# mklawonn/Scene-Graph-GAN

Hardware: AMD Instinct MI355X
Metric: triples/sec (G+D step) (higher is better)
Workload: dtype f32 (conv operands scaled per tensor and split into 2 fp16 pieces, round-to-nearest = 23 significant bits, 3 fp16 MFMAs per product, f32 accumulate; native-f32 figure and parity in the same line); 1 GPU; BASELINE.json configs[1] (1xMI355X, batch 64, 224x224, vocab 1000): batch 64 per GPU, 224x224 synthetic images, vocab 1000, 3-token triples, 1 critic update + 1 generator update per step (WGAN-GP lambda=10, TF-Adam); global_batch=64, critic_iters=1, parallelism=dp1, conv_precision_mode=2, schedule=two-stream; per-kernel figures from serial steps

## Files before the change

scene-graph-gan_amd/build.py:

```python
from __future__ import annotations

import hashlib
import os
import subprocess
import sys
from concurrent.futures import ThreadPoolExecutor

HERE = os.path.dirname(os.path.abspath(__file__))
CSRC = os.path.join(HERE, "csrc")
OUT_DIR = os.path.join(HERE, "_build")
LIB_PATH = os.path.join(HERE, "libsgg_hip.so")
ARCH = "gfx950"
HIPCC = os.environ.get("HIPCC", "/opt/rocm/bin/hipcc")
NO_PACKED_FP32 = ["-Xclang", "-target-feature", "-Xclang", "-packed-fp32-ops"]
FLAGS = ["-O3", "-std=c++17", "-fPIC", "--offload-arch=" + ARCH, "-fno-gpu-rdc", "-Wall", "-Wno-unused-function",
         "-ffp-contract=fast"] + NO_PACKED_FP32


def sources():
    return sorted(os.path.join(CSRC, f) for f in os.listdir(CSRC) if f.endswith(".hip"))


def _digest(paths):
    h = hashlib.sha256()
    for p in sorted(paths):
        with open(p, "rb") as f:
            h.update(p.encode())
            h.update(f.read())
    h.update(" ".join(FLAGS).encode())
    return h.hexdigest()


def _compile(src):
    obj = os.path.join(OUT_DIR, os.path.basename(src) + ".o")
    cmd = [HIPCC] + FLAGS + ["-I", CSRC, "-c", src, "-o", obj]
    r = subprocess.run(cmd, capture_output=True, text=True)
    if r.returncode != 0:
        raise RuntimeError("hipcc failed for %s:\n%s\n%s" % (src, r.stdout, r.stderr))
    err = "\n".join(l for l in r.stderr.splitlines() if "is not a recognized feature for this target" not in l)
    return obj, err


OBJDUMP = os.environ.get("LLVM_OBJDUMP", os.path.join(os.path.dirname(os.path.dirname(os.path.realpath(HIPCC))), "lib", "llvm", "bin",
                                                      "llvm-objdump"))


M0_ASM_KERNELS = ("conv_wgrad_dma", "conv_s2_kernel")


def check_device_code(lib_path: str = LIB_PATH) -> int:
    import re
    import shutil
    tmp = os.path.join(OUT_DIR, "disasm")
    shutil.rmtree(tmp, ignore_errors=True)
    os.makedirs(tmp)
    copy = os.path.join(tmp, "lib.so")
    shutil.copy(lib_path, copy)
    if not os.path.exists(OBJDUMP):
        raise RuntimeError("llvm-objdump not found at %s (set LLVM_OBJDUMP): the build cannot verify that the library is free of "
                           "packed-fp32 VALU instructions" % OBJDUMP)
    r = subprocess.run([OBJDUMP, "--offloading", copy], capture_output=True, text=True)
    if r.returncode != 0:
        raise RuntimeError("llvm-objdump --offloading failed:\n%s" % r.stderr)
    objs = sorted(f for f in os.listdir(tmp) if f.endswith(ARCH))
    if not objs:
        raise RuntimeError("no %s code object found in %s" % (ARCH, lib_path))
    pat, n_ins, bad = re.compile(r"\bv_pk_[a-z0-9]+_f32\b"), 0, []
    sym_pat = re.compile(r"^[0-9a-f]+ <(\S+)>:")
    m0_ok = re.compile(r"^\s*s_mov_b32 m0, s\d+\b")
    m0_implicit = re.compile(r"\b(v_movrel[sd]*_b32|s_movrel[sd]_b(32|64)|v_readlane_b32 \S+, \S+, m0|v_writelane_b32 \S+, \S+, m0|s_sendmsg|ds_gws_\w+|"
                             r"v_interp_\w+|s_load_\w+ .*\bm0\b)")
    m0_bad, m0_seen, cur = [], 0, ""
    for f in objs:
        d = subprocess.run([OBJDUMP, "-d", os.path.join(tmp, f)], capture_output=True, text=True)
        if d.returncode != 0:
            raise RuntimeError("llvm-objdump -d failed on %s:\n%s" % (f, d.stderr))
        for line in d.stdout.splitlines():
            m = sym_pat.match(line)
            if m:
                cur = m.group(1)
# ... 58 lines not shown
```

scene-graph-gan_amd/csrc/conv_halo.h:

```cpp
#pragma once
#include "sgg_common.h"

struct HaloParams {
  const float* src;
  const void* wfrag;
  const float* bias;
  float* out;
  const float* amax_src;
  const float* amax_w;
  float* tile_stats;
  const float* ln_stats;
  const float* ln_gamma;
  const float* ln_beta;
  int B, H, W, C, N;
  int bh, bw, nblk;
  int flip;
  unsigned src_bytes, w_bytes;
  int gx;
  int in_rs, in_ps, in_cA, in_cB;
  int out_rs, out_ps, out_nA, out_nB;
  int ln_nc;
  int frag16;
  int src_s16;
  int cu_cap;
// ... 16 lines not shown
int sgg_halo_pc64_applicable(int C, int N, int precision);
void sgg_halo_pc_launch(const HaloParams& p, int precision, hipStream_t st);

struct WgradHaloPlan {
  int ct, nt;
  int nbs;
  int spw;
  int pairs, pairs_n;
  int nsplit;
  int stages;
  int nslabs;
  int geo;
  int R, pc, xslots;
  size_t ws_bytes;
};
int sgg_wgrad_halo_plan(int B, int H, int W, int Cin, int Cout, int KH, int KW, int stride, WgradHaloPlan* pl);
void sgg_wgrad_halo_launch(const float* x, const float* dy, float* slabs, int B, int H, int W, int Cin, int Cout, int stride,
                           int pad_t, int pad_l, int precision, const float* amax_x, const float* amax_dy, const WgradHaloPlan& pl,
                           hipStream_t st, const float* ln_stats = nullptr, const float* ln_gamma = nullptr,
                           const float* ln_beta = nullptr, int operand_format = 0);

struct WgradDmaPlan {
  int nt;
  int spw;
  int pairs, pairs_n;
  int nsplit, stages, nslabs;
  int geo, R, pc, xslots;
  size_t ws_bytes;
};
int sgg_wgrad_dma_plan(int B, int H, int W, int Cin, int Cout, int KH, int KW, int stride, WgradDmaPlan* pl);
void sgg_wgrad_dma_launch(const void* x, const void* dy, float* slabs, int B, int H, int W, int Cin, int Cout, int stride, int pad_t,
                          int pad_l, const float* amax_x, const float* amax_dy, const WgradDmaPlan& pl, hipStream_t st);

struct S2Params {
  const float* src;
  const void* wfrag;
  const float* bias;
  float* out;
  const float* amax_src;
  const float* amax_w;
  float* tile_stats;
  const float* ln_stats;
  const float* ln_gamma;
  const float* ln_beta;
  int B, Ho, Wo;
  int C, N;
  int M;
  int nbands;
  int pitch;
  unsigned src_bytes, w_bytes;
  int gx;
  int src_s16;
  int ksplit;
  int cu_cap;
};
int sgg_s2_applicable(int KH, int KW, int stride, int B, int Hi, int Wi, int C, int N, int precision);
int sgg_s2_stats_per_sample(int Ho, int Wo, int N);
void sgg_s2_launch(const S2Params& p, int dgrad, int precision, hipStream_t st);
```

scene-graph-gan_amd/csrc/conv_wgrad.hip:

```cpp
#include "mma_f32.h"
#include "conv_halo.h"
#include <stdlib.h>

typedef __bf16 bf16x8 __attribute__((ext_vector_type(8)));
typedef __bf16 bf16x2 __attribute__((ext_vector_type(2)));
typedef float f32x2_t __attribute__((ext_vector_type(2)));
typedef unsigned u32x4 __attribute__((ext_vector_type(4)));

typedef _Float16 f16x8 __attribute__((ext_vector_type(8)));
typedef __fp16 fp16x2 __attribute__((ext_vector_type(2)));

template <int P, bool HALF>
__device__ __forceinline__ void split8_regs(const float (&x)[8], float scale, u32x4 (&pl)[P]) {
#pragma unroll
  for (int q = 0; q < 4; ++q) {
    float a = x[2 * q], b = x[2 * q + 1];
    if constexpr (HALF) {
      a *= scale; b *= scale;
      unsigned hi, lo;
      f16_split2(a, b, hi, lo);
      pl[0][q] = hi; pl[1][q] = lo;
    } else {
#pragma unroll
      for (int pp = 0; pp < P; ++pp) {
// ... 551 lines not shown
static WgradPlan wgrad_plan(int B, int Ho, int Wo, int Cin, int Cout, int KH, int KW) {
  WgradPlan pl;
  const long long mpix = (long long)B * Ho * Wo;
  if (Cin == 3) {
    pl.bmc = 27; pl.bnc = 32;
    pl.tiles = B * sgg_cdiv(Ho, 8) * sgg_cdiv(Wo, 32);
    pl.chunk = sgg_cdiv(pl.tiles, 1024);
    pl.nsplit = sgg_cdiv(pl.tiles, pl.chunk);
    pl.ws_bytes = (size_t)pl.nsplit * 27 * 32 * sizeof(float);
    return pl;
  }
  pl.bmc = Cin >= 128 ? 128 : Cin;
  pl.bnc = Cout >= 128 ? 128 : Cout;
  pl.tiles = (Cin / pl.bmc) * (Cout / pl.bnc);
  const int base = pl.tiles * KH * KW;
  int ns = (SGG_WGRAD_WGS + base - 1) / base;
  const long long max_ns = mpix / 512 > 0 ? mpix / 512 : 1;
  if (ns > max_ns) ns = (int)max_ns;
  if (ns < 1) ns = 1;
  pl.chunk = (int)(((mpix + ns - 1) / ns + 31) / 32 * 32);
  pl.nsplit = (int)((mpix + pl.chunk - 1) / pl.chunk);
  pl.ws_bytes = pl.nsplit > 1 ? (size_t)pl.nsplit * KH * KW * Cin * Cout * sizeof(float) : 0;
  return pl;
}

extern "C" size_t sgg_conv2d_nhwc_wgrad_workspace_bytes(int B, int Hi, int Wi, int Cin, int Ho, int Wo, int Cout, int KH,
                                                        int KW) {
  size_t need = wgrad_plan(B, Ho, Wo, Cin, Cout, KH, KW).ws_bytes;
  WgradHaloPlan hp;
  const int st_guess = (Hi == Ho && Wi == Wo) ? 1 : ((Hi == 2 * Ho && Wi == 2 * Wo) ? 2 : 0);
  if (st_guess && Cin != 3 && sgg_wgrad_halo_plan(B, Ho, Wo, Cin, Cout, KH, KW, st_guess, &hp) && hp.ws_bytes > need) need = hp.ws_bytes;
  WgradDmaPlan dp;
  if (st_guess && Cin != 3 && sgg_wgrad_dma_plan(B, Ho, Wo, Cin, Cout, KH, KW, st_guess, &dp) && dp.ws_bytes > need) need = dp.ws_bytes;
  return need;
}

extern "C" int sgg_conv2d_nhwc_wgrad_resident(int B, int Ho, int Wo, int Cin, int Cout, int KH, int KW, int stride, int precision) {
  WgradHaloPlan hp;
  if (!(sgg_prec_resident(precision) && Cin != 3 && B > 0 && sgg_wgrad_halo_plan(B, Ho, Wo, Cin, Cout, KH, KW, stride, &hp))) return 0;
  WgradDmaPlan dp;
  return (precision == 2 && sgg_wgrad_dma_plan(B, Ho, Wo, Cin, Cout, KH, KW, stride, &dp)) ? 2 : 1;
}

extern "C" int sgg_conv2d_nhwc_wgrad(const float* x, const float* dy, float* dw, int B, int Hi, int Wi, int Cin, int Ho,
                                     int Wo, int Cout, int KH, int KW, int stride, int pad_t, int pad_l, int precision, int algo,
                                     const float* amax_x, const float* amax_dy, const float* ln_stats, const float* ln_gamma,
                                     const float* ln_beta, int operand_format, void* workspace, size_t workspace_bytes, void* stream) {
  SGG_CHECK_ARG(x && dy && dw, "sgg_conv2d_nhwc_wgrad: null pointer");
  SGG_CHECK_ARG(operand_format >= 0 && operand_format <= 3 && (operand_format == 0 || (sgg_prec_half(precision) && Cin != 3 && algo == 0)) &&
                    !((operand_format & 1) && ln_stats),
                "sgg_conv2d_nhwc_wgrad: pre-split (S16) operands need precision 1 / 2 and the halo-resident kernel (algo 0); x with an LN "
                "prologue is the f32 pre-LayerNorm tensor");
  SGG_CHECK_ARG(!ln_stats || (ln_gamma && ln_beta), "sgg_conv2d_nhwc_wgrad: the LN prologue needs stats, gamma and beta");
  SGG_CHECK_ARG(algo == 0 || algo == 1, "sgg_conv2d_nhwc_wgrad: algo must be 0 (auto) or 1 (per-tap kernels only)");
  SGG_CHECK_ARG(precision == 0 || (precision >= 1 && precision <= 4) || precision == 6,
                "sgg_conv2d_nhwc_wgrad: precision must be 0, 1, 2, 3, 4 or 6");
  SGG_CHECK_ARG(!sgg_prec_half(precision) || Cin == 3 || (amax_x && amax_dy), "sgg_conv2d_nhwc_wgrad: precision 1 / 2 need the amax words");
  SGG_CHECK_ARG(!ln_stats || !sgg_prec_one(precision), "sgg_conv2d_nhwc_wgrad: the LN prologue exists in the two-piece modes (2, 3) only");
  SGG_CHECK_ARG(B > 0 && Hi > 0 && Wi > 0 && Ho > 0 && Wo > 0 && stride >= 1 && stride <= 2, "sgg_conv2d_nhwc_wgrad: bad dims");
  SGG_CHECK_ARG((long long)B * Hi * Wi * Cin < (1LL << 31) && (long long)B * Ho * Wo * Cout < (1LL << 31),
                "sgg_conv2d_nhwc_wgrad: tensor exceeds 2^31 elements");
  hipStream_t st = (hipStream_t)stream;
  const WgradPlan pl = wgrad_plan(B, Ho, Wo, Cin, Cout, KH, KW);
  if (pl.ws_bytes > 0) {
    if (!workspace || workspace_bytes < pl.ws_bytes) {
      sgg_set_error("sgg_conv2d_nhwc_wgrad: workspace too small (%zu < %zu)", workspace_bytes, pl.ws_bytes);
      return SGG_ERR_WORKSPACE;
    }
  }
  const long long nout = (long long)KH * KW * Cin * Cout;
  WgradDmaPlan dp;
  if (operand_format == 3 && precision == 2 && !ln_stats && algo == 0 && pad_t == 1 && pad_l == 1 && Hi == Ho * stride &&
      Wi == Wo * stride && sgg_wgrad_dma_plan(B, Ho, Wo, Cin, Cout, KH, KW, stride, &dp)) {
    if (!workspace || workspace_bytes < dp.ws_bytes) {
      sgg_set_error("sgg_conv2d_nhwc_wgrad: workspace too small (%zu < %zu)", workspace_bytes, dp.ws_bytes);
      return SGG_ERR_WORKSPACE;
    }
    sgg_wgrad_dma_launch(x, dy, (float*)workspace, B, Ho, Wo, Cin, Cout, stride, pad_t, pad_l, amax_x, amax_dy, dp, st);
    SGG_LAUNCH_CHECK("sgg_conv2d_nhwc_wgrad(dma)");
    launch_slab_reduce((const float*)workspace, dw, nout / 4, dp.nslabs, st);
    SGG_LAUNCH_CHECK("sgg_conv2d_nhwc_wgrad(dma reduce)");
    return SGG_OK;
  }
  WgradHaloPlan hp;
  if (sgg_prec_resident(precision) && Cin != 3 && pad_t == 1 && pad_l == 1 && Hi == Ho * stride && Wi == Wo * stride &&
      algo == 0 && sgg_wgrad_halo_plan(B, Ho, Wo, Cin, Cout, KH, KW, stride, &hp) && !(hp.geo == 1 && ln_stats)) {
    if (!workspace || workspace_bytes < hp.ws_bytes) {
      sgg_set_error("sgg_conv2d_nhwc_wgrad: workspace too small (%zu < %zu)", workspace_bytes, hp.ws_bytes);
      return SGG_ERR_WORKSPACE;
    }
    sgg_wgrad_halo_launch(x, dy, (float*)workspace, B, Ho, Wo, Cin, Cout, stride, pad_t, pad_l, precision, amax_x, amax_dy, hp, st,
                          ln_stats, ln_gamma, ln_beta, operand_format);
    SGG_LAUNCH_CHECK("sgg_conv2d_nhwc_wgrad(halo)");
    launch_slab_reduce((const float*)workspace, dw, nout / 4, hp.nslabs, st);
    SGG_LAUNCH_CHECK("sgg_conv2d_nhwc_wgrad(halo reduce)");
    return SGG_OK;
  }
  SGG_CHECK_ARG(operand_format == 0, "sgg_conv2d_nhwc_wgrad: pre-split (S16) operands are served by the halo-resident kernel only");
  SGG_CHECK_ARG(!ln_stats, "sgg_conv2d_nhwc_wgrad: the LN prologue is served by the halo-resident kernel only (3x3 stride 1 or 5x5 "
                           "stride 2 on grids divisible by 8, precision 2 or 3, algo 0)");
  if (Cin == 3) {
    SGG_CHECK_ARG(KH == 3 && KW == 3 && stride == 1 && Cout == 32, "sgg_conv2d_nhwc_wgrad: Cin=3 path needs 3x3 s1 Cout=32");
    hipLaunchKernelGGL(conv_c3_wgrad_kernel<false>, dim3(pl.nsplit), dim3(256), 0, st, x, dy, (float*)workspace, Hi, Wi, pad_t, pad_l,
                       sgg_cdiv(Wo, 32), sgg_cdiv(Ho, 8), pl.tiles, pl.chunk, C3LnArgs{nullptr, nullptr, nullptr, nullptr, nullptr, nullptr});
    SGG_LAUNCH_CHECK("sgg_conv2d_nhwc_wgrad(c3)");
    launch_slab_reduce((const float*)workspace, dw, nout / 4, pl.nsplit, st);
    SGG_LAUNCH_CHECK("sgg_conv2d_nhwc_wgrad(c3 reduce)");
    return SGG_OK;
  }
  SGG_CHECK_ARG(Cin % 32 == 0 && Cout % 32 == 0, "sgg_conv2d_nhwc_wgrad: Cin and Cout must be multiples of 32 (or Cin == 3)");
  SGG_CHECK_ARG(pl.bmc == 32 || pl.bmc == 64 || pl.bmc == 128, "sgg_conv2d_nhwc_wgrad: unsupported Cin tile");
  SGG_CHECK_ARG(pl.bnc == 32 || pl.bnc == 64 || pl.bnc == 128, "sgg_conv2d_nhwc_wgrad: unsupported Cout tile");
  WgradParams p;
  p.x = x; p.dy = dy; p.out = pl.nsplit > 1 ? (float*)workspace : dw;
// ... 62 lines not shown
```

scene-graph-gan_amd/csrc/conv_wgrad_dma.hip:

```cpp
#include "split16.h"
#include "conv_halo.h"
#include <type_traits>

typedef short wd_s16x4 __attribute__((ext_vector_type(4)));
typedef unsigned wd_u32x2 __attribute__((ext_vector_type(2)));
typedef __attribute__((address_space(3))) void* wd_lds_ptr;

typedef int wd_v4i __attribute__((ext_vector_type(4)));
__device__ __forceinline__ void wd_dma16(wd_v4i rs, unsigned lds_addr, unsigned voff, int soff) {
  asm volatile("s_mov_b32 m0, %0\n\ts_nop 0\n\tbuffer_load_dwordx4 %1, %2, %3 offen lds"
               :
               : "s"(lds_addr), "v"(voff), "s"(rs), "s"(soff)
               : "memory");
}
__device__ __forceinline__ wd_v4i wd_rsrc(const void* base, unsigned bytes) {
  const unsigned long long a = reinterpret_cast<unsigned long long>(base);
  return wd_v4i{(int)(unsigned)a, (int)((unsigned)(a >> 32) & 0xffffu), (int)bytes, 0x00020000};
}
__device__ __forceinline__ unsigned wd_lds_addr(const unsigned char* p) {
  return (unsigned)(unsigned long long)(__attribute__((address_space(3))) const unsigned char*)p;
}

__device__ __forceinline__ wd_u32x2 wd_tr16(const unsigned char* p) {
  return __builtin_bit_cast(wd_u32x2, __builtin_amdgcn_ds_read_tr16_b64_v4i16((__attribute__((address_space(3))) wd_s16x4*)p));
}

struct WgradDmaParams {
  const void* x;
  const void* dy;
  float* slabs;
  const float* amax_x;
  const float* amax_dy;
  int B, H, W, C, N;
  int Hx, Wx, sxy, cy, cx, a0y, a0x, kh0, kw0, kstep, KWt, taps_total;
  int bh, bw, nblk;
  int pairs_n;
  int stages;
  unsigned x_bytes, dy_bytes;
};

#define WD_XSUB 8192
#define WD_XPLANE (2 * WD_XSUB)
#define WD_DSUB 4096

template <int NT, int NKH, int NKW>
__global__ __launch_bounds__(512, 2) void conv_wgrad_dma_kernel(WgradDmaParams p) {
  static_assert(NT == 4 || NT == 2, "64 x 128 or 64 x 64 channel tiles");
  constexpr int NTAP = NKH * NKW;
  constexpr int DPLANE = NT * WD_DSUB;
  constexpr int BUF = 2 * WD_XPLANE + 2 * DPLANE;
  constexpr int KSW = NT == 4 ? 4 : 2;
  constexpr int SPW = NT == 4 ? 1 : 2;
  __shared__ __attribute__((aligned(1024))) unsigned char lds[2 * BUF];

// ... 363 lines not shown
```

scene-graph-gan_amd/lib.py:

```python
from __future__ import annotations

import ctypes
import os
from ctypes import c_char_p, c_float, c_int, c_longlong, c_size_t, c_void_p

import torch

_HERE = os.path.dirname(os.path.abspath(__file__))
LIB_PATH = os.path.join(_HERE, "libsgg_hip.so")

_vp, _i, _f, _sz, _ll = c_void_p, c_int, c_float, c_size_t, c_longlong

SIGNATURES = {
    "sgg_version": (_i, []),
    "sgg_last_error": (c_char_p, []),
    "sgg_device_info": (_i, [_vp, _vp, _vp, _vp, _i]),
    "sgg_hwio_to_hwoi": (_i, [_vp, _vp, _i, _i, _i, _vp]),
    "sgg_conv_split_weights": (_i, [_vp, _vp, _ll, _i, _vp, _vp]),
    "sgg_absmax": (_i, [_vp, _ll, _vp, _vp]),
    "sgg_conv_wsplit_layout": (_i, [_i] * 8),
    "sgg_conv_wsplit_layout_presplit": (_i, [_i] * 8),
    "sgg_conv_s2d_weights": (_i, [_vp, _vp, _i, _i, _vp]),
    "sgg_conv_prepare_weights": (_i, [_vp, _i, _i, _vp]),
    "sgg_conv_split_weights_frag": (_i, [_vp, _vp, _i, _i, _i, _i, _vp, _vp]),
# ... 66 lines not shown
        return _lib
    path = os.environ.get("SGG_HIP_LIB", path)
    if not os.path.exists(path):
        raise SggError("libsgg_hip.so not found at %s - run `python -c 'import __graft_entry__ as g; g.build()'` "
                       "(there is no CPU fallback)" % path)
    lib = ctypes.CDLL(path)
    for name, (res, args) in SIGNATURES.items():
        fn = getattr(lib, name)
        fn.restype = res
        fn.argtypes = args
    _lib = lib
    return lib


def same_pads(in_size: int, k: int, s: int):
    out = -(-in_size // s)
    total = max((out - 1) * s + k - in_size, 0)
    return out, total // 2, total - total // 2


def _p(t):
    return None if t is None else t.data_ptr()


def _ld(t):
    return t.stride(0) if t.shape[0] > 1 else max(t.stride(0), t.shape[1])


DEFAULT_OPTIONS = {
    "conv_precision": 2,
    "conv_halo": True,
    "halo_pc": True,
    "halo_pc64": True,
    "ln_fusion": 1,
    "presplit": True,
    "presplit_head_grad": True,
    "wgrad_late": True,
    "side_priority": 0,
    "g_early": 1,
    "g_early_cus": 28,
    "c3_ln_bwd_fused": True,
    "d_side_cus": 0,
    "fwd_cus": 0,
    "ln_fusion_skip": (),
    "ln_fusion_force": (),
    "ln_fusion_force_bwd": (),
    "ln_fusion_skip_bwd": (),
}


def options_from_env(base=None):
    opts = dict(DEFAULT_OPTIONS if base is None else base)
    for item in filter(None, os.environ.get("SGG_OPTIONS", "").split(",")):
        key, _, val = item.partition("=")
        key = key.strip()
        if key not in DEFAULT_OPTIONS:
            raise SggError("SGG_OPTIONS: unknown option %r (known: %s)" % (key, ", ".join(sorted(DEFAULT_OPTIONS))))
        d = DEFAULT_OPTIONS[key]
        if isinstance(d, bool):
            opts[key] = val.strip().lower() not in ("0", "false", "no", "off", "")
        elif isinstance(d, tuple):
            opts[key] = tuple(int(v) for v in val.split("+") if v.strip())
        else:
            opts[key] = int(val)
    return opts

# ... 200 lines not shown
        else:
            nb = 4.0 * (x.numel() + y.numel())
        self._check(self._timed(sym, flops, lambda: self.lib.sgg_conv2d_nhwc_fwd(
            _p(x), _p(w_fwd), _p(w_split), _p(bias), _p(y), *d, self.conv_precision, w_split_layout, _p(amax_x), _p(amax_w),
            _p(tile_stats), _p(ln_s), _p(ln_g), _p(ln_b), int(bool(x_s16)) | ((int(cu_cap) & 63) << 8), self._stream()), nb),
            "sgg_conv2d_nhwc_fwd")

    def conv_dgrad(self, dy, w_hwio, dx, stride, w_split=None, amax_dy=None, amax_w=None, w_split_layout=0, dy_s16=False):
        self._dev(dy, w_hwio, dx)
        d = self._conv_dims(dx.shape, w_hwio.shape, stride)
        assert tuple(dy.shape) == (d[0], d[4], d[5], d[6]) and dy.is_contiguous() and dx.is_contiguous()
        flops = 2.0 * d[0] * d[4] * d[5] * d[6] * d[7] * d[8] * d[3]
        amax_dy, amax_w = self._amax_or_compute(dy, amax_dy, 0), self._amax_or_compute(w_hwio, amax_w, 1)
        sym = self.halo_pc_symbol(False, dy_s16, d[3]) if w_split_layout == 4 else self.halo_symbol(d[3], d[6]) if w_split_layout == 1 else (self.halo_symbol(4 * d[3], d[6]) if w_split_layout == 3 else
                                                                          self.s2_symbol(True, d[0] * d[4] * d[5], d[3], False, False, dy_s16) if w_split_layout == 2 else
                                                                          self.gather_symbol(d[3], w_split is not None))
        self._check(self._timed(sym, flops, lambda: self.lib.sgg_conv2d_nhwc_dgrad(
            _p(dy), _p(w_hwio), _p(w_split), _p(dx), *d, self.conv_precision, w_split_layout, _p(amax_dy), _p(amax_w),
            int(bool(dy_s16)), self._stream())), "sgg_conv2d_nhwc_dgrad")

    def wgrad_resident(self, B, Ho, Wo, cin, cout, k, stride):
        return bool(self.conv_halo and self.lib.sgg_conv2d_nhwc_wgrad_resident(B, Ho, Wo, cin, cout, k, k, stride, self.conv_precision))

    def conv_wgrad(self, x, dy, dw, stride, amax_x=None, amax_dy=None, ln=None, x_s16=False, dy_s16=False):
        self._dev(x, dy, dw)
        ln_s, ln_g, ln_b = ln if ln is not None else (None, None, None)
        self._dev(ln_s, ln_g, ln_b)
        d = self._conv_dims(x.shape, dw.shape, stride)
        assert tuple(dy.shape) == (d[0], d[4], d[5], d[6]) and x.is_contiguous() and dy.is_contiguous() and dw.is_contiguous()
        need = self.lib.sgg_conv2d_nhwc_wgrad_workspace_bytes(*d[:9])
        ws = self.workspace(need)
        flops = 2.0 * d[0] * d[4] * d[5] * d[6] * d[7] * d[8] * d[3]
        sym, nb = "conv_wgrad(call: wgrad kernel + slab reduce)", 0.0
        if x_s16 and dy_s16 and ln is None and self.conv_precision == 2 and self.conv_halo and \
                self.lib.sgg_conv2d_nhwc_wgrad_resident(d[0], d[4], d[5], d[3], d[6], d[7], d[8], stride, 2) == 2:
            sym = "conv_wgrad_dma(call: LDS-DMA kernel on pre-split operands + slab reduce)"
        if d[3] != 3:
            amax_x, amax_dy = self._amax_or_compute(x, amax_x, 0), self._amax_or_compute(dy, amax_dy, 1)
        else:
            sym, nb = "conv_c3_wgrad(call: kernel + slab reduce)", 4.0 * (x.numel() + dy.numel())
        self._check(self._timed(sym, flops, lambda: self.lib.sgg_conv2d_nhwc_wgrad(
            _p(x), _p(dy), _p(dw), *d, self.conv_precision, 0 if self.conv_halo else 1, _p(amax_x), _p(amax_dy), _p(ln_s), _p(ln_g), _p(ln_b),
            int(bool(x_s16)) | (int(bool(dy_s16)) << 1), _p(ws), ws.numel(), self._stream()), nb),
            "sgg_conv2d_nhwc_wgrad")

    @staticmethod
    def _region(region, H, W):
        if region is None:
            return (0, 0, 0, 0, 0)
        y0, x0, hv, wv = region
        assert 0 <= y0 and 0 <= x0 and y0 + hv <= H and x0 + wv <= W, (region, H, W)
        return (W, y0, x0, hv, wv)

    def ln_elu_fwd(self, y, gamma, beta, a, stats, amax_out=None, tile_stats=None, region=None, out_s16=False):
        self._dev(y, gamma, beta, a, stats, amax_out, tile_stats)
        B, H, W, C = y.shape
        assert region is None or tile_stats is None
        need = self.lib.sgg_layernorm_hwc_elu_workspace_bytes(B, H * W, C)
        ws = self.workspace(need)
        nts = 0 if tile_stats is None else tile_stats.shape[1]
        nb = 4.0 * y.numel() * (2 if nts else 3)
        self._check(self._timed("ln_elu_fwd(call)", 0.0, lambda: self.lib.sgg_layernorm_hwc_elu_fwd(
            _p(y), _p(gamma), _p(beta), _p(a), _p(stats), _p(amax_out), _p(tile_stats), nts, B, H * W, C,
            *self._region(region, H, W), int(bool(out_s16)), _p(ws), ws.numel(), self._stream()), nb), "sgg_layernorm_hwc_elu_fwd")

    def ln_finalize(self, tile_stats, gamma, beta, stats, amax_out, hw):
        self._dev(tile_stats, gamma, beta, stats, amax_out)
        B, nts, _ = tile_stats.shape
        self._check(self.lib.sgg_layernorm_hwc_finalize(_p(tile_stats), nts, _p(gamma), _p(beta), _p(stats), _p(amax_out), B, hw,
                                                        gamma.shape[0], self._stream()), "sgg_layernorm_hwc_finalize")

    def ln_prologue_ok(self, k, stride, H, W, cin, cout):
        if not (self.conv_halo and self.conv_precision in (2, 3) and cin <= 512):
            return False
        lay = self.lib.sgg_conv_wsplit_layout(k, k, stride, H, W, cin, cout, self.conv_precision)
        return lay in (1, 3, 4) or (lay == 2 and (H // 2) % 8 == 0 and (W // 2) % 8 == 0)
# ... 308 lines not shown
```

Measured before the change: 1521 triples/sec.

## Add producer/consumer wgrad kernel fusing LN-ELU prologue with LDS-DMA dy staging

Adds a warp-specialized weight-gradient kernel. Four producer waves load raw x, apply the LayerNorm+ELU prologue, split it into fp16 pieces and write it to LDS, and DMA pre-split dy into a 4-deep ring. Four consumer waves run the 3-MFMA split products at high priority. It replaces the halo-resident path for LN-fused wgrad with pre-split dy and pad 1, aiming to overlap operand preparation with MFMA work. In exchange it adds a large new kernel with fixed LDS layouts and more slab workspace.

Result: no change. 1529 triples/sec, median of 6 (+0.5%).

```diff
diff --git a/scene-graph-gan_amd/build.py b/scene-graph-gan_amd/build.py
--- a/scene-graph-gan_amd/build.py
+++ b/scene-graph-gan_amd/build.py
@@ -45,7 +45,7 @@
                                                       "llvm-objdump"))
 
 
-M0_ASM_KERNELS = ("conv_wgrad_dma", "conv_s2_kernel")
+M0_ASM_KERNELS = ("conv_wgrad_dma", "conv_wgrad_pc", "conv_s2_kernel")
 
 
 def check_device_code(lib_path: str = LIB_PATH) -> int:
diff --git a/scene-graph-gan_amd/csrc/conv_halo.h b/scene-graph-gan_amd/csrc/conv_halo.h
--- a/scene-graph-gan_amd/csrc/conv_halo.h
+++ b/scene-graph-gan_amd/csrc/conv_halo.h
@@ -72,6 +72,19 @@
 void sgg_wgrad_dma_launch(const void* x, const void* dy, float* slabs, int B, int H, int W, int Cin, int Cout, int stride, int pad_t,
                           int pad_l, const float* amax_x, const float* amax_dy, const WgradDmaPlan& pl, hipStream_t st);
 
+struct WgradPcPlan {
+  int ct;
+  int nbs;
+  int spw;
+  int pairs, pairs_n;
+  int nsplit, stages, nslabs;
+  size_t ws_bytes;
+};
+int sgg_wgrad_pc_plan(int B, int H, int W, int Cin, int Cout, int KH, int KW, int stride, WgradPcPlan* pl);
+void sgg_wgrad_pc_launch(const float* x, const void* dy, float* slabs, int B, int H, int W, int Cin, int Cout, int stride, int pad_t,
+                         int pad_l, const float* amax_x, const float* amax_dy, const float* ln_stats, const float* ln_gamma,
+                         const float* ln_beta, const WgradPcPlan& pl, hipStream_t st);
+
 struct S2Params {
   const float* src;
   const void* wfrag;
diff --git a/scene-graph-gan_amd/csrc/conv_wgrad.hip b/scene-graph-gan_amd/csrc/conv_wgrad.hip
--- a/scene-graph-gan_amd/csrc/conv_wgrad.hip
+++ b/scene-graph-gan_amd/csrc/conv_wgrad.hip
@@ -607,6 +607,8 @@
   if (st_guess && Cin != 3 && sgg_wgrad_halo_plan(B, Ho, Wo, Cin, Cout, KH, KW, st_guess, &hp) && hp.ws_bytes > need) need = hp.ws_bytes;
   WgradDmaPlan dp;
   if (st_guess && Cin != 3 && sgg_wgrad_dma_plan(B, Ho, Wo, Cin, Cout, KH, KW, st_guess, &dp) && dp.ws_bytes > need) need = dp.ws_bytes;
+  WgradPcPlan pp;
+  if (st_guess && Cin != 3 && sgg_wgrad_pc_plan(B, Ho, Wo, Cin, Cout, KH, KW, st_guess, &pp) && pp.ws_bytes > need) need = pp.ws_bytes;
   return need;
 }
 
@@ -614,7 +616,9 @@
   WgradHaloPlan hp;
   if (!(sgg_prec_resident(precision) && Cin != 3 && B > 0 && sgg_wgrad_halo_plan(B, Ho, Wo, Cin, Cout, KH, KW, stride, &hp))) return 0;
   WgradDmaPlan dp;
-  return (precision == 2 && sgg_wgrad_dma_plan(B, Ho, Wo, Cin, Cout, KH, KW, stride, &dp)) ? 2 : 1;
+  WgradPcPlan pp;
+  return ((precision == 2 && sgg_wgrad_dma_plan(B, Ho, Wo, Cin, Cout, KH, KW, stride, &dp)) ? 2 : 1) |
+         ((precision == 2 && hp.geo == 0 && sgg_wgrad_pc_plan(B, Ho, Wo, Cin, Cout, KH, KW, stride, &pp)) ? 4 : 0);
 }
 
 extern "C" int sgg_conv2d_nhwc_wgrad(const float* x, const float* dy, float* dw, int B, int Hi, int Wi, int Cin, int Ho,
@@ -622,6 +626,8 @@
                                      const float* amax_x, const float* amax_dy, const float* ln_stats, const float* ln_gamma,
                                      const float* ln_beta, int operand_format, void* workspace, size_t workspace_bytes, void* stream) {
   SGG_CHECK_ARG(x && dy && dw, "sgg_conv2d_nhwc_wgrad: null pointer");
+  const bool no_pc = operand_format >= 0 && (operand_format & 4);
+  if (operand_format >= 0) operand_format &= ~4;
   SGG_CHECK_ARG(operand_format >= 0 && operand_format <= 3 && (operand_format == 0 || (sgg_prec_half(precision) && Cin != 3 && algo == 0)) &&
                     !((operand_format & 1) && ln_stats),
                 "sgg_conv2d_nhwc_wgrad: pre-split (S16) operands need precision 1 / 2 and the halo-resident kernel (algo 0); x with an LN "
@@ -655,6 +661,20 @@
     SGG_LAUNCH_CHECK("sgg_conv2d_nhwc_wgrad(dma)");
     launch_slab_reduce((const float*)workspace, dw, nout / 4, dp.nslabs, st);
     SGG_LAUNCH_CHECK("sgg_conv2d_nhwc_wgrad(dma reduce)");
+    return SGG_OK;
+  }
+  WgradPcPlan pp;
+  if (operand_format == 2 && precision == 2 && ln_stats && algo == 0 && !no_pc && pad_t == 1 && pad_l == 1 && Hi == Ho * stride &&
+      Wi == Wo * stride && sgg_wgrad_pc_plan(B, Ho, Wo, Cin, Cout, KH, KW, stride, &pp)) {
+    if (!workspace || workspace_bytes < pp.ws_bytes) {
+      sgg_set_error("sgg_conv2d_nhwc_wgrad: workspace too small (%zu < %zu)", workspace_bytes, pp.ws_bytes);
+      return SGG_ERR_WORKSPACE;
+    }
+    sgg_wgrad_pc_launch(x, dy, (float*)workspace, B, Ho, Wo, Cin, Cout, stride, pad_t, pad_l, amax_x, amax_dy, ln_stats, ln_gamma, ln_beta,
+                        pp, st);
+    SGG_LAUNCH_CHECK("sgg_conv2d_nhwc_wgrad(pc)");
+    launch_slab_reduce((const float*)workspace, dw, nout / 4, pp.nslabs, st);
+    SGG_LAUNCH_CHECK("sgg_conv2d_nhwc_wgrad(pc reduce)");
     return SGG_OK;
   }
   WgradHaloPlan hp;
diff --git a/scene-graph-gan_amd/csrc/conv_wgrad_dma.hip b/scene-graph-gan_amd/csrc/conv_wgrad_dma.hip
--- a/scene-graph-gan_amd/csrc/conv_wgrad_dma.hip
+++ b/scene-graph-gan_amd/csrc/conv_wgrad_dma.hip
@@ -1,25 +1,10 @@
 #include "split16.h"
 #include "conv_halo.h"
+#include "lds_dma.h"
 #include <type_traits>
 
 typedef short wd_s16x4 __attribute__((ext_vector_type(4)));
 typedef unsigned wd_u32x2 __attribute__((ext_vector_type(2)));
-typedef __attribute__((address_space(3))) void* wd_lds_ptr;
-
-typedef int wd_v4i __attribute__((ext_vector_type(4)));
-__device__ __forceinline__ void wd_dma16(wd_v4i rs, unsigned lds_addr, unsigned voff, int soff) {
-  asm volatile("s_mov_b32 m0, %0\n\ts_nop 0\n\tbuffer_load_dwordx4 %1, %2, %3 offen lds"
-               :
-               : "s"(lds_addr), "v"(voff), "s"(rs), "s"(soff)
-               : "memory");
-}
-__device__ __forceinline__ wd_v4i wd_rsrc(const void* base, unsigned bytes) {
-  const unsigned long long a = reinterpret_cast<unsigned long long>(base);
-  return wd_v4i{(int)(unsigned)a, (int)((unsigned)(a >> 32) & 0xffffu), (int)bytes, 0x00020000};
-}
-__device__ __forceinline__ unsigned wd_lds_addr(const unsigned char* p) {
-  return (unsigned)(unsigned long long)(__attribute__((address_space(3))) const unsigned char*)p;
-}
 
 __device__ __forceinline__ wd_u32x2 wd_tr16(const unsigned char* p) {
   return __builtin_bit_cast(wd_u32x2, __builtin_amdgcn_ds_read_tr16_b64_v4i16((__attribute__((address_space(3))) wd_s16x4*)p));
diff --git a/scene-graph-gan_amd/csrc/conv_wgrad_pc.hip b/scene-graph-gan_amd/csrc/conv_wgrad_pc.hip
--- /dev/null
+++ b/scene-graph-gan_amd/csrc/conv_wgrad_pc.hip
@@ -0,0 +1,344 @@
+#include "split16.h"
+#include "conv_halo.h"
+#include "lds_dma.h"
+#include <type_traits>
+
+typedef short wp_s16x4 __attribute__((ext_vector_type(4)));
+typedef unsigned wp_u32x2 __attribute__((ext_vector_type(2)));
+
+__device__ __forceinline__ wp_u32x2 wp_tr16(const unsigned char* p) {
+  return __builtin_bit_cast(wp_u32x2, __builtin_amdgcn_ds_read_tr16_b64_v4i16((__attribute__((address_space(3))) wp_s16x4*)p));
+}
+constexpr int wp_wait(int n) { return (n & 15) | ((n >> 4) << 14) | 0x0070; }
+
+struct WgradPcParams {
+  const float* x;
+  const void* dy;
+  float* slabs;
+  const float* amax_x;
+  const float* amax_dy;
+  const float* ln_stats;
+  const float* ln_gamma;
+  const float* ln_beta;
+  int B, H, W, C, N;
+  int Hx, Wx, sxy, cy, cx, a0y, a0x, kh0, kw0, kstep, KWt, taps_total;
+  int bh, bw, nblk;
+  int pairs_n;
+  int stages;
+  unsigned x_bytes, dy_bytes;
+};
+
+#define WP_XSUB 7680
+#define WP_XPLANE (2 * WP_XSUB)
+#define WP_XSTAGE (2 * WP_XPLANE)
+#define WP_DSUB 4096
+#define WP_DPLANE (2 * WP_DSUB)
+#define WP_DSTAGE (2 * WP_DPLANE)
+#define WP_DRING 4
+#define WP_XOFF (WP_DRING * WP_DSTAGE)
+#define WP_LNOFF (WP_XOFF + 2 * WP_XSTAGE)
+
+template <int CT, int NKH, int NKW>
+__global__ __launch_bounds__(512, 2) void conv_wgrad_pc_kernel(WgradPcParams p) {
+  static_assert(CT == 1 || CT == 2, "32 x 32 or 64 x 64 channel chunks");
+  constexpr int NT = CT;
+  constexpr int NTAP = NKH * NKW;
+  constexpr int NBS = CT == 2 ? 1 : 2;
+  constexpr int KSW = CT == 2 ? 4 : 2;
+  constexpr int SPW = CT == 2 ? 1 : 4;
+  constexpr int XI = 400 * CT, XP = (XI + 255) / 256;
+  constexpr int NIT = NBS * XP;
+  __shared__ __attribute__((aligned(1024))) unsigned char lds[WP_LNOFF + 512];
+  float* const lnp_s = reinterpret_cast<float*>(lds + WP_LNOFF);
+
+  const int tid = threadIdx.x, lane = tid & 63;
+  const int wave = __builtin_amdgcn_readfirstlane(tid >> 6);
+  const int split = blockIdx.x, pair = blockIdx.y;
+  const int c0 = (pair / p.pairs_n) * 32 * CT, n0 = (pair % p.pairs_n) * 32 * NT;
+  if (tid < 32 * CT) {
+    lnp_s[tid] = p.ln_gamma[c0 + tid];
+    lnp_s[32 * CT + tid] = p.ln_beta[c0 + tid];
+  }
+  __syncthreads();
+  const int ea = scale_exp_from_amax(*p.amax_x), eb = scale_exp_from_amax(*p.amax_dy);
+
+  if (wave >= 4) {
+    const int pw = wave - 4, ptid = tid - 256;
+    const __amdgpu_buffer_rsrc_t rs_x = __builtin_amdgcn_make_buffer_rsrc(const_cast<float*>(p.x), 0, p.x_bytes, 0x00020000);
+    const wd_v4i rs_dy = wd_rsrc(p.dy, p.dy_bytes);
+    const float sa = ldexpf(1.f, ea);
+    unsigned it_rel[NIT];
+    int it_lds[NIT];
+#pragma unroll
+    for (int j = 0; j < NIT; ++j) {
+      const int blk = j / XP, i = ptid + 256 * (j % XP);
+      const int csub = i / 400, r = i % 400;
+      const int px = r >> 2, c4 = r & 3;
+      const int ry = px / 10, rx = px % 10;
+      it_rel[j] = (unsigned)(((ry * p.sxy * p.Wx + rx * p.sxy) * p.C + csub * 32 + c4 * 8) * 4);
+      const int bits = (ry == 0) | ((ry == 9) << 1) | ((rx == 0) << 2) | ((rx == 9) << 3);
+      it_lds[j] = ((blk * CT + csub) * WP_XSUB + (ry * 12 + rx) * 64 + c4 * 16) | (bits << 20) | ((i < XI) << 24);
+    }
+    float it_g[NIT][8], it_b[NIT][8];
+#pragma unroll
+    for (int j = 0; j < NIT; ++j) {
+      const int i = ptid + 256 * (j % XP);
+      const int cbx = (i < XI ? i / 400 : 0) * 32 + ((i % 400) & 3) * 8;
+#pragma unroll
+      for (int c = 0; c < 8; ++c) { it_g[j][c] = lnp_s[cbx + c]; it_b[j][c] = lnp_s[32 * CT + cbx + c]; }
+    }
+    const int dpx = 16 * pw + (lane >> 2);
+    const unsigned drel = (unsigned)((((dpx >> 3) * p.W + (dpx & 7)) * p.N) * 4 + (lane & 3) * 16);
+
+    const int bpi = p.bh * p.bw;
+    const int blk_begin = split * p.stages * NBS, blk_end = blk_begin + p.stages * NBS;
+    int cb[NBS], cy[NBS], cx[NBS];
+#pragma unroll
+    for (int j = 0; j < NBS; ++j) {
+      const int beta = blk_begin + j;
+      cb[j] = beta / bpi;
+      const int rem = beta % bpi;
+      cy[j] = rem / p.bw;
+      cx[j] = rem % p.bw;
+    }
+    int next_beta = blk_begin;
+    unsigned f_xbase[NBS], f_dbase[NBS];
+    int f_bbits[NBS];
+    bool f_dead[NBS];
+    float f_mu[NBS], f_rs[NBS];
+    auto fetch_plan = [&]() __attribute__((always_inline)) {
+#pragma unroll
+      for (int blk = 0; blk < NBS; ++blk) {
+        f_dead[blk] = (next_beta + blk >= p.nblk) | (next_beta + blk >= blk_end);
+        const int by = cy[blk], bx = cx[blk];
+        f_xbase[blk] = (unsigned)((((cb[blk] * p.Hx + (by * 8 - 1) * p.sxy + p.cy) * p.Wx + (bx * 8 - 1) * p.sxy + p.cx) * p.C + c0) * 4);
+        f_dbase[blk] = (unsigned)((((cb[blk] * p.H + by * 8) * p.W + bx * 8) * p.N + n0) * 4);
+        f_bbits[blk] = (by == 0) | ((by == p.bh - 1) << 1) | ((bx == 0) << 2) | ((bx == p.bw - 1) << 3);
+        const int b = cb[blk] < p.B ? cb[blk] : p.B - 1;
+        f_mu[blk] = p.ln_stats[2 * b];
+        f_rs[blk] = p.ln_stats[2 * b + 1];
+        cx[blk] += NBS;
+        while (cx[blk] >= p.bw) {
+          cx[blk] -= p.bw;
+          if (++cy[blk] >= p.bh) { cy[blk] = 0; ++cb[blk]; }
+        }
+      }
+      next_beta += NBS;
+    };
+    f32x4 pre[2][NIT][2];
+    int m_bad[2] = {0, 0};
+    float m_mu[2][NBS], m_rs[2][NBS];
+    auto load_item = [&](auto set_c, int j) __attribute__((always_inline)) {
+      constexpr int S = decltype(set_c)::value;
+      const int blk = j / XP;
+      const bool bad = f_dead[blk] | !((it_lds[j] >> 24) & 1) | (((it_lds[j] >> 20) & 15 & f_bbits[blk]) != 0);
+      m_bad[S] |= (int)bad << j;
+      const unsigned off = bad ? SGG_OOB : f_xbase[blk] + it_rel[j];
+      pre[S][j][0] = buf_load4(rs_x, off);
+      pre[S][j][1] = buf_load4(rs_x, off + 16u);
+    };
+    auto keep_stats = [&](auto set_c) __attribute__((always_inline)) {
+      constexpr int S = decltype(set_c)::value;
+      m_bad[S] = 0;
+#pragma unroll
+      for (int blk = 0; blk < NBS; ++blk) { m_mu[S][blk] = f_mu[blk]; m_rs[S][blk] = f_rs[blk]; }
+    };
+    auto dma_dy = [&](unsigned char* dbuf) __attribute__((always_inline)) {
+      const unsigned dd = wd_lds_addr(dbuf) + pw * 1024;
+#pragma unroll
+      for (int sub = 0; sub < 2; ++sub) {
+        const int blk = CT == 2 ? 0 : sub;
+        const unsigned dof = f_dead[blk] ? SGG_OOB : f_dbase[blk] + drel;
+        const int soff = CT == 2 ? sub * 128 : 0;
+        wd_dma16(rs_dy, dd + sub * WP_DSUB, dof, soff);
+        wd_dma16(rs_dy, dd + WP_DPLANE + sub * WP_DSUB, dof, soff + 64);
+      }
+    };
+    int d_i = 0;
+    auto stage = [&](auto set_c) __attribute__((always_inline)) {
+      constexpr int S = decltype(set_c)::value;
+      unsigned char* xw = lds + WP_XOFF + S * WP_XSTAGE;
+      const int c_bad = m_bad[S];
+      float c_mu[NBS], c_rs[NBS];
+#pragma unroll
+      for (int blk = 0; blk < NBS; ++blk) { c_mu[blk] = m_mu[S][blk]; c_rs[blk] = m_rs[S][blk]; }
+      fetch_plan();
+      keep_stats(set_c);
+      dma_dy(lds + d_i * WP_DSTAGE);
+      d_i = (d_i + 1) & (WP_DRING - 1);
+#pragma unroll
+      for (int j = 0; j < NIT; ++j) {
+        const int blk = j / XP;
+        ln_elu8(pre[S][j][0], pre[S][j][1], it_g[j], it_b[j], c_mu[blk], c_rs[blk], (c_bad >> j) & 1);
+        u32x4 pl[2];
+        split8<2, true>(pre[S][j][0], pre[S][j][1], sa, pl);
+        if ((it_lds[j] >> 24) & 1) {
+          unsigned char* dst = xw + (it_lds[j] & 0xfffff);
+          *reinterpret_cast<u32x4*>(dst) = pl[0];
+          *reinterpret_cast<u32x4*>(dst + WP_XPLANE) = pl[1];
+        }
+        load_item(set_c, j);
+      }
+      __builtin_amdgcn_sched_barrier(0);
+      __builtin_amdgcn_s_waitcnt(wp_wait(2 * (2 * NIT + 4)));
+      __builtin_amdgcn_s_barrier();
+    };
+    using set0 = std::integral_constant<int, 0>;
+    using set1 = std::integral_constant<int, 1>;
+
+    fetch_plan();
+    keep_stats(set0{});
+    dma_dy(lds);
+#pragma unroll
+    for (int j = 0; j < NIT; ++j) load_item(set0{}, j);
+    fetch_plan();
+    keep_stats(set1{});
+    dma_dy(lds + WP_DSTAGE);
+#pragma unroll
+    for (int j = 0; j < NIT; ++j) load_item(set1{}, j);
+    d_i = 2;
+    for (int t = 0; t <= p.stages; t += 2) {
+      stage(set0{});
+      if (t + 1 <= p.stages) stage(set1{});
+    }
+    __builtin_amdgcn_s_waitcnt(wp_wait(0));
+    return;
+  }
+
+  int ci_t, co_t, wblk, ks0, sw;
+  if constexpr (CT == 2) { ci_t = wave >> 1; co_t = wave & 1; wblk = 0; ks0 = 0; sw = 0; }
+  else { ci_t = 0; co_t = 0; wblk = wave >> 1; ks0 = 2 * (wave & 1); sw = wave; }
+  const int g = lane >> 4, q = (lane >> 2) & 3, pch = lane & 3;
+  const int choff = ((g & 1) * 2 + (pch >> 1)) * 16 + (pch & 1) * 8;
+  const int a_off = WP_XOFF + (wblk * CT + ci_t) * WP_XSUB + ((2 * ks0 + (g >> 1) + p.a0y + 1) * 12 + q + p.a0x + 1) * 64 + choff;
+  const int b_off = (wblk * NT + co_t) * WP_DSUB + ((2 * ks0 + (g >> 1)) * 8 + q) * 64 + choff;
+
+  f32x16 acc[NTAP];
+#pragma unroll
+  for (int t = 0; t < NTAP; ++t)
+#pragma unroll
+    for (int r = 0; r < 16; ++r) acc[t][r] = 0.f;
+
+  auto compute = [&](const unsigned char* a_base, const unsigned char* b_base) __attribute__((always_inline)) {
+    constexpr int NS = KSW * NTAP;
+    u32x4 a[3][2], b[2][2];
+    auto rd_b = [&](int ksi, u32x4 (&o)[2]) __attribute__((always_inline)) {
+#pragma unroll
+      for (int pp = 0; pp < 2; ++pp) {
+        const wp_u32x2 lo = wp_tr16(b_base + (2 * ksi * 8) * 64 + pp * WP_DPLANE);
+        const wp_u32x2 hi = wp_tr16(b_base + (2 * ksi * 8 + 4) * 64 + pp * WP_DPLANE);
+        o[pp] = u32x4{lo[0], lo[1], hi[0], hi[1]};
+      }
+    };
+    auto rd_a = [&](int step, u32x4 (&o)[2]) __attribute__((always_inline)) {
+      const int ksi = step / NTAP, tap = step % NTAP;
+      const int kh = tap / NKW, kw = tap % NKW;
+#pragma unroll
+      for (int pp = 0; pp < 2; ++pp) {
+        const wp_u32x2 lo = wp_tr16(a_base + ((2 * ksi + kh) * 12 + kw) * 64 + pp * WP_XPLANE);
+        const wp_u32x2 hi = wp_tr16(a_base + ((2 * ksi + kh) * 12 + kw + 4) * 64 + pp * WP_XPLANE);
+        o[pp] = u32x4{lo[0], lo[1], hi[0], hi[1]};
+      }
+    };
+    rd_b(0, b[0]);
+    rd_a(0, a[0]);
+    rd_a(1, a[1]);
+#pragma unroll
+    for (int step = 0; step < NS; ++step) {
+      const int ksi = step / NTAP, tap = step % NTAP;
+      if (step + 2 < NS) rd_a(step + 2, a[(step + 2) % 3]);
+      if (tap == 0 && ksi + 1 < KSW) rd_b(ksi + 1, b[(ksi + 1) & 1]);
+      f32x16 d = acc[tap];
+      d = mfma16<true>(a[step % 3][1], b[ksi & 1][0], d);
+      d = mfma16<true>(a[step % 3][0], b[ksi & 1][1], d);
+      d = mfma16<true>(a[step % 3][0], b[ksi & 1][0], d);
+      acc[tap] = d;
+      __builtin_amdgcn_sched_barrier(0);
+    }
+  };
+
+  __builtin_amdgcn_s_barrier();
+  int c_i = 0;
+  for (int s = 0; s < p.stages; ++s) {
+    SGG_PRIO_HI();
+    compute(lds + a_off + (s & 1) * WP_XSTAGE, lds + b_off + c_i * WP_DSTAGE);
+    SGG_PRIO_LO();
+    c_i = (c_i + 1) & (WP_DRING - 1);
+    __builtin_amdgcn_sched_barrier(0);
+    __builtin_amdgcn_s_waitcnt(wp_wait(63));
+    __builtin_amdgcn_s_barrier();
+  }
+
+  float* o = p.slabs + (size_t)(split * SPW + sw) * p.taps_total * p.C * p.N;
+#pragma unroll
+  for (int tap = 0; tap < NTAP; ++tap)
+#pragma unroll
+    for (int r = 0; r < 16; ++r) {
+      const int ci = c0 + ci_t * 32 + acc_row(r, lane);
+      const int co = n0 + co_t * 32 + acc_col(lane);
+      const int ktap = (p.kh0 + p.kstep * (tap / NKW)) * p.KWt + p.kw0 + p.kstep * (tap % NKW);
+      o[((size_t)ktap * p.C + ci) * p.N + co] = ldexpf(ldexpf(acc[tap][r], -ea), -eb);
+    }
+}
+
+int sgg_wgrad_pc_plan(int B, int H, int W, int Cin, int Cout, int KH, int KW, int stride, WgradPcPlan* pl) {
+  const bool k3 = KH == 3 && KW == 3 && stride == 1, k5 = KH == 5 && KW == 5 && stride == 2;
+  if (!((k3 || k5) && B > 0 && H > 0 && W > 0 && H % 8 == 0 && W % 8 == 0)) return 0;
+  if ((size_t)B * H * W * stride * stride * Cin * sizeof(float) >= 0x80000000ull || (size_t)B * H * W * Cout * sizeof(float) >= 0x80000000ull)
+    return 0;
+  if (Cin == 32 && Cout == 32) pl->ct = 1;
+  else if (Cin > 0 && Cout > 0 && Cin % 64 == 0 && Cout % 64 == 0) pl->ct = 2;
+  else return 0;
+  pl->nbs = pl->ct == 2 ? 1 : 2;
+  pl->spw = pl->ct == 2 ? 1 : 4;
+  pl->pairs_n = Cout / (32 * pl->ct);
+  pl->pairs = (Cin / (32 * pl->ct)) * pl->pairs_n;
+  const int nblk = B * (H / 8) * (W / 8);
+  const int total_stages = (nblk + pl->nbs - 1) / pl->nbs;
+  int ns = 256 / pl->pairs;
+  if (ns > total_stages / 4) ns = total_stages / 4;
+  if (ns < 1) ns = 1;
+  pl->stages = (total_stages + ns - 1) / ns;
+  pl->nsplit = (total_stages + pl->stages - 1) / pl->stages;
+  pl->nslabs = pl->nsplit * pl->spw;
+  pl->ws_bytes = (size_t)pl->nslabs * KH * KW * Cin * Cout * sizeof(float);
+  return 1;
+}
+
+template <int NKH, int NKW>
+static void wgrad_pc_launch_class(const WgradPcParams& p, const WgradPcPlan& pl, hipStream_t st) {
+  const dim3 grid(pl.nsplit, pl.pairs);
+  if (pl.ct == 2) hipLaunchKernelGGL((conv_wgrad_pc_kernel<2, NKH, NKW>), grid, dim3(512), 0, st, p);
+  else hipLaunchKernelGGL((conv_wgrad_pc_kernel<1, NKH, NKW>), grid, dim3(512), 0, st, p);
+}
+
+void sgg_wgrad_pc_launch(const float* x, const void* dy, float* slabs, int B, int H, int W, int Cin, int Cout, int stride, int pad_t,
+                         int pad_l, const float* amax_x, const float* amax_dy, const float* ln_stats, const float* ln_gamma,
+                         const float* ln_beta, const WgradPcPlan& pl, hipStream_t st) {
+  WgradPcParams p;
+  p.x = x; p.dy = dy; p.slabs = slabs; p.amax_x = amax_x; p.amax_dy = amax_dy;
+  p.ln_stats = ln_stats; p.ln_gamma = ln_gamma; p.ln_beta = ln_beta;
+  p.B = B; p.H = H; p.W = W; p.C = Cin; p.N = Cout; p.bh = H / 8; p.bw = W / 8; p.nblk = B * p.bh * p.bw;
+  p.Hx = H * stride; p.Wx = W * stride; p.sxy = stride;
+  p.pairs_n = pl.pairs_n; p.stages = pl.stages;
+  p.x_bytes = (unsigned)((size_t)B * p.Hx * p.Wx * Cin * sizeof(float));
+  p.dy_bytes = (unsigned)((size_t)B * H * W * Cout * sizeof(float));
+  if (stride == 1) {
+    p.cy = p.cx = 0; p.a0y = p.a0x = -1; p.kh0 = p.kw0 = 0; p.kstep = 1; p.KWt = 3; p.taps_total = 9;
+    wgrad_pc_launch_class<3, 3>(p, pl, st);
+    return;
+  }
+  p.kstep = 2; p.KWt = 5; p.taps_total = 25;
+  for (int cy = 0; cy < 2; ++cy)
+    for (int cx = 0; cx < 2; ++cx) {
+      const int kh0 = (pad_t + cy) % 2, kw0 = (pad_l + cx) % 2;
+      p.cy = cy; p.cx = cx; p.kh0 = kh0; p.kw0 = kw0;
+      p.a0y = (kh0 - pad_t - cy) / 2;
+      p.a0x = (kw0 - pad_l - cx) / 2;
+      const int nkh = (5 - kh0 + 1) / 2, nkw = (5 - kw0 + 1) / 2;
+      if (nkh == 3 && nkw == 3) wgrad_pc_launch_class<3, 3>(p, pl, st);
+      else if (nkh == 3) wgrad_pc_launch_class<3, 2>(p, pl, st);
+      else if (nkw == 3) wgrad_pc_launch_class<2, 3>(p, pl, st);
+      else wgrad_pc_launch_class<2, 2>(p, pl, st);
+    }
+}
diff --git a/scene-graph-gan_amd/csrc/lds_dma.h b/scene-graph-gan_amd/csrc/lds_dma.h
--- /dev/null
+++ b/scene-graph-gan_amd/csrc/lds_dma.h
@@ -0,0 +1,19 @@
+#pragma once
+#include "sgg_common.h"
+
+typedef __attribute__((address_space(3))) void* wd_lds_ptr;
+
+typedef int wd_v4i __attribute__((ext_vector_type(4)));
+__device__ __forceinline__ void wd_dma16(wd_v4i rs, unsigned lds_addr, unsigned voff, int soff) {
+  asm volatile("s_mov_b32 m0, %0\n\ts_nop 0\n\tbuffer_load_dwordx4 %1, %2, %3 offen lds"
+               :
+               : "s"(lds_addr), "v"(voff), "s"(rs), "s"(soff)
+               : "memory");
+}
+__device__ __forceinline__ wd_v4i wd_rsrc(const void* base, unsigned bytes) {
+  const unsigned long long a = reinterpret_cast<unsigned long long>(base);
+  return wd_v4i{(int)(unsigned)a, (int)((unsigned)(a >> 32) & 0xffffu), (int)bytes, 0x00020000};
+}
+__device__ __forceinline__ unsigned wd_lds_addr(const unsigned char* p) {
+  return (unsigned)(unsigned long long)(__attribute__((address_space(3))) const unsigned char*)p;
+}
diff --git a/scene-graph-gan_amd/lib.py b/scene-graph-gan_amd/lib.py
--- a/scene-graph-gan_amd/lib.py
+++ b/scene-graph-gan_amd/lib.py
@@ -122,6 +122,7 @@
     "conv_halo": True,
     "halo_pc": True,
     "halo_pc64": True,
+    "wgrad_pc": True,
     "ln_fusion": 1,
     "presplit": True,
     "presplit_head_grad": True,
@@ -388,16 +389,21 @@
         ws = self.workspace(need)
         flops = 2.0 * d[0] * d[4] * d[5] * d[6] * d[7] * d[8] * d[3]
         sym, nb = "conv_wgrad(call: wgrad kernel + slab reduce)", 0.0
-        if x_s16 and dy_s16 and ln is None and self.conv_precision == 2 and self.conv_halo and \
-                self.lib.sgg_conv2d_nhwc_wgrad_resident(d[0], d[4], d[5], d[3], d[6], d[7], d[8], stride, 2) == 2:
+        res = self.lib.sgg_conv2d_nhwc_wgrad_resident(d[0], d[4], d[5], d[3], d[6], d[7], d[8], stride, 2) \
+            if self.conv_precision == 2 and self.conv_halo and d[3] != 3 else 0
+        if x_s16 and dy_s16 and ln is None and (res & 3) == 2:
             sym = "conv_wgrad_dma(call: LDS-DMA kernel on pre-split operands + slab reduce)"
+        no_pc = not getattr(self, "wgrad_pc", True)
+        if ln is not None and dy_s16 and not x_s16 and (res & 4) and not no_pc and d[10] == 1 and d[11] == 1 and \
+                d[1] == d[4] * stride and d[2] == d[5] * stride:
+            sym = "conv_wgrad_pc(call: producer/consumer kernel, LN prologue + pre-split dy + slab reduce)"
         if d[3] != 3:
             amax_x, amax_dy = self._amax_or_compute(x, amax_x, 0), self._amax_or_compute(dy, amax_dy, 1)
         else:
             sym, nb = "conv_c3_wgrad(call: kernel + slab reduce)", 4.0 * (x.numel() + dy.numel())
         self._check(self._timed(sym, flops, lambda: self.lib.sgg_conv2d_nhwc_wgrad(
             _p(x), _p(dy), _p(dw), *d, self.conv_precision, 0 if self.conv_halo else 1, _p(amax_x), _p(amax_dy), _p(ln_s), _p(ln_g), _p(ln_b),
-            int(bool(x_s16)) | (int(bool(dy_s16)) << 1), _p(ws), ws.numel(), self._stream()), nb),
+            int(bool(x_s16)) | (int(bool(dy_s16)) << 1) | (4 if no_pc else 0), _p(ws), ws.numel(), self._stream()), nb),
             "sgg_conv2d_nhwc_wgrad")
 
     @staticmethod
```
